# zengxianyu/sketchedit

Measured on AMD Instinct MI355X. Metric: images/sec, higher is better.
Workload: dtype f32; 1 GPU; SketchEdit inference forward (netM+netG, use_cam, pool max) 256x256 batch 32 per GPU, procedural weights; global_batch=32, size=256, per_gpu_batch=32, execution=default, two streams

## Files before the change

sketchedit_amd/csrc/se_kernels.h:

```cpp
#pragma once
#include <hip/hip_runtime.h>
#include <stddef.h>
#include <stdint.h>

#include <vector>

struct se_window;

namespace se {

enum ProfLabel { PL_GCONV_N192 = 0, PL_GCONV_N96, PL_GCONV_N48, PL_GCONV_N24, PL_WINO_N192, PL_WINO_N96, PL_WINO_UP96, PL_SMALL_CONV, PL_PACK, PL_COLREDUCE,
                 PL_ATT_PREP, PL_ATT_SCORE, PL_ATT_SOFTMAX, PL_ATT_BOXSUM, PL_ATT_PV, PL_LAYOUT,
                 PL_ATT_STREAM_STATS, PL_ATT_STREAM_OUT, PL_RESIZE_H, PL_RESIZE_V, PL_WINDOW_GATHER, PL_WINDOW_BORDER, PL_WINDOW_PASTE,
                 PL_WINDOW_RESAMPLE_H, PL_WINDOW_PASTE_V, PL_WINDOW_SAVE, PL_WINDOW_SWAP, PL_WINDOW_LOCK_GATHER, PL_WINDOW_PASTE_LOCKED,
                 PL_WINDOW_PASTE_V_LOCKED, PL_SKETCH_TILES, PL_SKETCH_STROKES, PL_PNG_ROWS, PL_PNG_STRIPES,
                 PL_PNG_FINISH, PL_JPG_BLOCKS, PL_JPG_ROWS, PL_JPG_FINISH, PL_JPG2_BLOCKS, PL_JPG2_HIST, PL_JPG2_TABLES,
                 PL_WINDOW_PASTE_FEATHER, PL_FILL_MASKS, PL_FILL_KEEP, PL_BLEND_INIT, PL_BLEND_PULL, PL_BLEND_RELAX, PL_BLEND_APPLY, PL_CANVAS_MAP, PL_CANVAS_TURN,
                 PL_SELECT_SIMILAR, PL_SELECT_FLOOD, PL_SELECT_GROW, PL_MODIFY_DISC, PL_MODIFY_VOTE,
                 PL_LASSO_FILL, PL_PLANE_COMBINE, PL_ADJUST, PL_HIST_TILES, PL_HIST_SUM, PL_ADJUST_LUT, PL_OUTLINE_COUNT, PL_OUTLINE_SCAN, PL_OUTLINE_EMIT, PL_FILTER_BLUR, PL_FILTER_MOSAIC, PL_MOVE_DROP,
                 PL_PLANE_SHIFT, PL_WARP_DROP, PL_PLANE_WARP, PL_COUNT };
const char* prof_label_name(int l);
struct Profiler {
  struct Rec { int label; const char* name; const char* form; double flops; double exec_flops; double bytes; long blocks; hipEvent_t a, b; };
  std::vector<Rec> recs;
  std::vector<hipEvent_t> pool;
  size_t used = 0;
  bool on = false;
};
void set_profiler(Profiler* p);
void set_launch_cost(double flops, double bytes, const char* name = nullptr, double exec_flops = -1.0);
void set_launch_grid(long blocks);
hipError_t ensure_max_lds(const void* func, int bytes);

#define SE_OPTIONS(X)                                                                                         \
  X(XCD_REMAP, 1)                                                             \
  X(RTILE, 1)                                              \
  X(RTILE_LL_MIN, 256)         \
  X(RTILE_WX, 2)          \
  X(RTILE_DENSE, 1)                                          \
  X(RTILE_D5W, 1)                                        \
  X(TEST_OFFSET_LIMIT, 0)  \
  X(TEST_POISON, 0)       \
  X(RCONV16, 1) X(RCONV16_DUAL, 1) X(RCONV96, 1) X(VECBIAS, 1)                                                  \
  X(WINOGRAD, 1) X(WINOGRAD48, 1) X(WINOGRAD_UP, 1) X(WINOGRAD_UP48, 1)                                         \
  X(WINOGRAD_F43, 1)      \
  X(S2_POLY, 1)           \
  X(GCONV_FAST, 1) X(FORK_DEFAULT, 1) X(LL_WINO_MIN_WG, 64) X(LL_WINO48_MIN_WG, 128)                            \
  X(ATT_FUSED, -1) X(ATT_FUSED_BF16, -1) X(ATT_PTILDE_LDS, 1) X(ATT_STATS_LDS, 1) X(ATT_E16, 1) X(ATT_SYM, 1)   \
  X(ATT_STREAM, 0)        \
  X(PAIR_MIN_PIXELS, 1 << 21)
enum Opt {
#define X(name, dflt) OPT_##name,
  SE_OPTIONS(X)
#undef X
  OPT_COUNT
};
int opt(int o);
int opt_set(const char* name, int value);
int opt_get(const char* name, int* value);
void opt_reset();
long long opt_epoch();

struct GConvParams {
  const float* src0;
  const float* src1;
  const float* wpk;
  const float* bias;
  float* dst;
  const float* zeros;
  int B, Hin, Win, Ho, Wo;
  int C0, C1;
  int C0g, CG;
  int T, KW;
  int magicCG, magicKW;
  int magicKH;
  unsigned rep;
  unsigned div_hw_m, div_w_m;
  int div_hw_l, div_w_l;
  int stride, dil, pad;
  int ushift;
  int up2;
  int OH, OW;
  int Hlim, Wlim;
  int src1_vec;
  int nch;
  int G;
  int act;
  int total_pix;
  int xcd;
  int np_full;
  int nf_full;
  int bf16;
  int small_grid;
};

static inline void udiv_magic_host(unsigned d, unsigned* m, int* l) {
  int ll = 0;
  while ((1ull << ll) < d) ++ll;
  *l = ll;
  *m = (unsigned)(((1ull << 32) * ((1ull << ll) - d)) / d + 1);
}

enum GConvCfg { GC_N192 = 0, GC_N96 = 1, GC_N48 = 2, GC_N24 = 3 };
static inline int gconv_np(int cfg) { return cfg == GC_N192 ? 192 : cfg == GC_N96 ? 96 : cfg == GC_N48 ? 48 : 32; }
static inline bool gconv_mixed(int cfg) { return cfg >= GC_N48; }

hipError_t launch_gconv(int cfg, const GConvParams& p, hipStream_t st);

struct WinoParams {
  const float* src;
  const float* src1;
  int src1_vec;
  const float* upk;
  const float* bias;
  float* dst;
  int B, h, w, d;
  int th, tw;
  int total_tiles;
  int act;
  int xcd;
  unsigned div_tpi_m, div_tw_m, div_d_m;
  int div_tpi_l, div_tw_l, div_d_l;
  const float* vbias;
};
hipError_t launch_wino(const WinoParams& p, hipStream_t st);
hipError_t launch_vecbias(const float* wv, const float* vec, float* T, int B, int C1, hipStream_t st, int round_vec = 0);
hipError_t launch_wino24(const WinoParams& p, hipStream_t st);
hipError_t launch_wino24_c48(const WinoParams& p, hipStream_t st);
hipError_t launch_wino48(const WinoParams& p, hipStream_t st);
hipError_t launch_wino48_c24(const WinoParams& p, hipStream_t st);
hipError_t launch_winoup(const WinoParams& p, hipStream_t st);
hipError_t launch_winoup48(const WinoParams& p, hipStream_t st);
hipError_t launch_s2poly48(const WinoParams& p, int halves, hipStream_t st);

struct RConvParams {
  const void* src;
  const void* wpk;
  const float* bias;
  void* dst;
  int B, h, w, d;
  int hs, ws;
  int ty, tx;
  int act;
  int xcd;
  const float* vbias;
  int dual;
};
hipError_t launch_rconv16(const RConvParams& p, hipStream_t st);

struct RConv96Params {
  const void* src;
  const void* wpk;
  const float* bias;
  void* dst;
  int B, h, w;
  int CG;
  int ty, tx;
  int stride, oh, ow;
  int up2;
  int act;
  int xcd;
};
hipError_t launch_rconv96(const RConv96Params& p, hipStream_t st);

struct RTileParams {
  const float* src;
  const float* wpk;
  const float* bias;
  float* dst;
  int B, Hin, Win;
  int C;
  int CG;
  int T, KW;
  int magicCG, magicKW;
  int pad;
  int up2, OH, OW;
  int G;
  int nch, NP;
  int RH, RW;
  int raw_bytes;
  unsigned div_cg_m, div_rw_m;
  int div_cg_l, div_rw_l;
  int ty, tx;
  int act, bf16, xcd;
  int dense;
};
hipError_t launch_rtile(const RTileParams& p, hipStream_t st);
hipError_t launch_rtilew(const RTileParams& p, hipStream_t st);
hipError_t launch_rtilew2(const RTileParams& p, hipStream_t st);
int rtile_rows(bool bf16);

struct SmallConvParams {
  const float* x;
  const float* w;
  const float* b;
  int B, H, W, cout;
  int mode;
  float* out_nchw;
  float* hard;
  const float* img;
  const float* mask;
  float* xnow;
  float* composed;
  int no_mask_coarse;
  long out_bs;
  long mask_bs;
  long comp_bs;
  int bf16;
  unsigned char* rgb8;
  unsigned char* m8;
  const unsigned char* lock;
  int raw_fine;
};
hipError_t launch_small_conv(const SmallConvParams& p, hipStream_t st);

hipError_t launch_pack_m(const float* image, const float* sketch, float* dst4, int B, int H, int W, hipStream_t st);
hipError_t launch_pack_g(const float* x, const float* x2, const float* mask, const float* mask2, const float* guide,
                         float* coarse8, float* style8, int B, int H, int W, int no_mask_cc, int joint,
                         hipStream_t st);
hipError_t launch_nchw_to_nhwc(const float* src, float* dst, int B, int C, int Cpad, int H, int W, hipStream_t st);
hipError_t launch_dequantize_u8(const unsigned char* rgb, const unsigned char* sk8, const float* lut, float* image, float* sketch,
                                int B, int H, int W, hipStream_t st);
hipError_t launch_nhwc_to_nchw(const float* src, float* dst, int B, int C, int Cstride, int H, int W, hipStream_t st);
hipError_t launch_quantize_u8(const float* composed, const float* mask, unsigned char* rgb, unsigned char* m8, int B, int H,
                              int W, hipStream_t st);
hipError_t launch_colreduce(const float* x, float* partial, float* out, int B, int HW, int C, int op, hipStream_t st,
                            int x_bf16 = 0, float* out_bf16 = nullptr);
hipError_t launch_pack_m16(const float* image, const float* sketch, float* dst8, int B, int H, int W, hipStream_t st);
hipError_t launch_pack_g16(const float* x, const float* x2, const float* mask, const float* mask2, const float* guide,
                           float* coarse8, float* style8, int B, int H, int W, int no_mask_cc, int joint, hipStream_t st);
hipError_t launch_nchw_to_nhwc16(const float* src, float* dst, int B, int C, int Cpad, int H, int W, hipStream_t st);
hipError_t launch_nhwc16_to_nchw(const float* src, float* dst, int B, int C, int Cstride, int H, int W, hipStream_t st);
static const int COLREDUCE_SPLITS = 128;

struct AttParams {
  const float* x;
  const float* rn;
  float* xn;
  const float* hard;
  float* valid;
  float* S;
  float* out;
  int B, h, w, hs, ws, L, Lp;
  float scale;
  float th;
  int hc, wc, R, Rp;
  float* xT;
  float* E;
  float* P;
  float* Pt;
  float* stats;
  float* kmul;
  float* kadd;
  int guard;
  float* validR;
  float* similar;
  int bf16;
  int e16;
  float* emean;
  float* epart;
  float* ea;
  float* eb;
  float* ea4;
  float* kadd2;
  int sym;
  int symT;
};
hipError_t launch_attention(const AttParams& p, hipStream_t st);
hipError_t launch_att2_prep(const AttParams& p, hipStream_t st);
hipError_t launch_attention_stream(const AttParams& p, hipStream_t st);
int att_stream_xt_tail();

int resample_ksize(int in, int out, int filter);
int resample_coeffs(int in, int out, int filter, int* bounds, int* kk);
enum { RESIZE_OUT_U8 = 0, RESIZE_OUT_IMAGE_F32 = 1, RESIZE_OUT_SKETCH_F32 = 2, RESIZE_OUT_LOCK_U8 = 3 };
struct ResizeOut {
  int mode;
  unsigned char* u8;
  float* f32;
  const float* lut;
  int H, W;
};
hipError_t launch_resample_h(const unsigned char* in, const int* d_bounds, const int* d_kk, const int* h_bounds, int ksize,
                             int B, int Hrows, int Win, int Wout, int C, const ResizeOut& o, hipStream_t st);
hipError_t launch_resample_v(const unsigned char* in, const int* d_bounds, const int* d_kk, int ksize, int B, int Hin, int Hout,
                             int W, int C, const ResizeOut& o, hipStream_t st);
hipError_t launch_window_resample_h(const se_window* d_wins, const int* d_bounds, const int* d_kk, const int* h_bounds, int ksize,
                                    int B, int hs, int ws, int Wout, int C, const ResizeOut& o, hipStream_t st);
hipError_t launch_window_paste_v(const se_window* d_wins, const unsigned char* rgb, const unsigned char* m8, const int* d_bounds,
                                 const int* d_kk, int ksize, int B, int Hin, int hs, int P, int ws, hipStream_t st, bool locked = false);
hipError_t launch_window_lock_resample_h(const se_window* d_wins, const int* d_bounds, const int* d_kk, const int* h_bounds, int ksize,
                                         int B, int hs, int ws, int Wout, const ResizeOut& o, hipStream_t st);
constexpr int RESAMPLE_MAX_KSIZE = 8191;

hipError_t launch_window_gather(const se_window* d_wins, const float* lut, float* image, float* sketch, int B, int H, int W,
                                hipStream_t st);
hipError_t launch_window_border(const se_window* d_wins, const unsigned char* m8, int* hits, int B, int H, int W, int hs, int ws,
                                hipStream_t st);
hipError_t launch_window_paste(const se_window* d_wins, const unsigned char* rgb, const unsigned char* m8, int B, int H, int W,
                               hipStream_t st, bool locked = false);
hipError_t launch_window_paste_feather(const se_window* d_wins, const unsigned char* rgb, const unsigned char* m8, int B, int hs, int ws,
                                       int radius, hipStream_t st);
hipError_t launch_window_lock_gather(const se_window* d_wins, unsigned char* out, int B, int H, int W, hipStream_t st);
hipError_t launch_window_journal(const se_window* d_wins, int B, int hs, int ws, bool swap, hipStream_t st);
hipError_t launch_sketch_tiles(const unsigned char* plane, int Hi, int Wi, int tile, int* tiles_out, hipStream_t st);
hipError_t launch_sketch_strokes(const se_window* d_wins, int B, int hs, int ws, const int* segs, long nseg_sum, unsigned char* sketch_out,
                                 hipStream_t st);
hipError_t launch_fill_masks(const unsigned char* fill, const unsigned char* lock, float* hole, float* hard, float* zero, int B, int H,
                             int W, hipStream_t st);
hipError_t launch_fill_keep(const se_window* d_wins, int B, int hs, int ws, hipStream_t st);
hipError_t launch_select_similar(const unsigned char* frame, int Hi, int Wi, int seed_y, int seed_x, int tolerance, int contiguous,
                                 unsigned char* state, hipStream_t st);
hipError_t launch_select_flood(unsigned char* state, int Hi, int Wi, unsigned* changed, hipStream_t st);
hipError_t launch_select_grow(const unsigned char* state, int Hi, int Wi, int grow, unsigned char* out, hipStream_t st);
hipError_t launch_plane_modify(const unsigned char* plane, int Hi, int Wi, int op, int radius, unsigned char* out, hipStream_t st);
hipError_t launch_lasso_fill(const int* edges, int N, int Hi, int Wi, unsigned char* plane_out, hipStream_t st);
hipError_t launch_plane_combine(const unsigned char* a, const unsigned char* b, int Hi, int Wi, int op, unsigned char* out, hipStream_t st);
hipError_t launch_outline_count(const unsigned char* plane, int Hi, int Wi, int* cnt, hipStream_t st);
hipError_t launch_outline_scan(int* cnt, int Hi, int Wi, int cap, int* info_out, hipStream_t st);
hipError_t launch_outline_emit(const unsigned char* plane, int Hi, int Wi, const int* offs, int* edges_out, int cap, hipStream_t st);
hipError_t launch_move_drop(unsigned char* frame, int Hi, int Wi, const unsigned char* lift, int ly0, int lx0, int lw, int lpitch,
                            const unsigned char* sel, const unsigned char* lock, int by0, int bx0, int by1, int bx1, int dy, int dx, int flip,
                            int radius, hipStream_t st);
hipError_t launch_plane_shift(const unsigned char* sel, int Hi, int Wi, int by0, int bx0, int by1, int bx1, int dy, int dx, int flip,
                              unsigned char* out, hipStream_t st);
size_t blend_workspace_bytes(int eh, int ew);
hipError_t launch_move_blend(unsigned char* frame, int Hi, int Wi, const unsigned char* lift, int ly0, int lx0, int lh, int lw, int lpitch,
                             const unsigned char* sel, const unsigned char* lock, int by0, int bx0, int by1, int bx1, int dy, int dx, int flip,
                             void* ws, hipStream_t st);
hipError_t launch_canvas(const unsigned char* in, int Hi, int Wi, int C, unsigned char* out, int Hn, int Wn, int oy, int ox, int orient,
                         int pad, unsigned rgb, hipStream_t st);
hipError_t launch_filter_blur(unsigned char* frame, int Hi, int Wi, const unsigned char* lift, int ly0, int lx0, int lw, int lpitch,
                              const unsigned char* sel, const unsigned char* lock, int by0, int bx0, int by1, int bx1, const int* taps,
                              int radius, int amount, int feather, hipStream_t st);
hipError_t launch_filter_mosaic(unsigned char* frame, int Hi, int Wi, const unsigned char* lift, int ly0, int lx0, int lw, int lpitch,
                                const unsigned char* sel, const unsigned char* lock, int by0, int bx0, int by1, int bx1, int cell, int amount,
                                int feather, hipStream_t st);
int adjust_hist_groups(int bh, int bw);
hipError_t launch_adjust(unsigned char* frame, int Hi, int Wi, const unsigned char* lift, int ly0, int lx0, int lw, int lpitch,
                         const unsigned char* sel, const unsigned char* lock, int by0, int bx0, int by1, int bx1, const unsigned char* lut,
                         const int* matrix, int amount, int feather, hipStream_t st);
hipError_t launch_hist_tiles(const unsigned char* frame, int Wi, const unsigned char* sel, int by0, int bx0, int by1, int bx1, unsigned* slabs,
                             hipStream_t st);
hipError_t launch_hist_sum(const unsigned* slabs, int groups, unsigned* hist, hipStream_t st);
hipError_t launch_adjust_lut(const unsigned* hist_src, const unsigned* hist_ref, int mode, int which, int clip, unsigned char* lut, hipStream_t st);
hipError_t launch_warp_drop(unsigned char* frame, int Hi, int Wi, const unsigned char* lift, int ly0, int lx0, int lw, int lpitch,
                            const unsigned char* sel, const unsigned char* lock, int by0, int bx0, int by1, int bx1, int ry0, int rx0,
                            int rh, int rw, const long long* m, hipStream_t st);
hipError_t launch_plane_warp(const unsigned char* sel, int Hi, int Wi, int by0, int bx0, int by1, int bx1, const long long* m,
                             unsigned char* out, hipStream_t st);
int png_stripes(int hs);
size_t png_stripe_bound(size_t n);
size_t png_slot_bytes(int ws);
hipError_t launch_png_rows(const se_window* d_wins, int B, int hs, int ws, unsigned char* ftype, hipStream_t st);
hipError_t launch_png_stripes(const se_window* d_wins, int B, int hs, int ws, const unsigned char* ftype, unsigned* sizes, unsigned* parts,
                              unsigned char* slots, hipStream_t st);
hipError_t launch_png_finish(int B, int hs, int ws, const unsigned* sizes, const unsigned* parts, const unsigned char* slots, unsigned char* out,
                             size_t cap, unsigned long long* sizes_out, hipStream_t st);
int jpg_rows(int hs, int flags);
int jpg_row_blocks(int ws, int flags);
size_t jpg_row_bound(int nblk, int flags);
size_t jpg_slot_bytes(int nblk, int flags);
hipError_t launch_jpg_blocks(const se_window* d_wins, int B, int hs, int ws, int quality, short* coef, hipStream_t st);
hipError_t launch_jpg2_blocks420(const se_window* d_wins, int B, int hs, int ws, int quality, short* coef, hipStream_t st);
hipError_t launch_jpg2_hist(int B, int R, int nblk, int flags, const short* coef, unsigned* hist, hipStream_t st);
hipError_t launch_jpg2_tables(int B, int R, const unsigned* hist, unsigned* codes, unsigned char* tables_out, hipStream_t st);
hipError_t launch_jpg_rows(int B, int R, int nblk, int flags, const short* coef, const unsigned* codes, unsigned* sizes,
                           unsigned char* slots, hipStream_t st);
hipError_t launch_jpg_finish(int B, int R, int nblk, size_t slot_bytes, const unsigned* sizes, const unsigned char* slots,
                             unsigned char* out, size_t cap, unsigned long long* sizes_out, hipStream_t st);

}
```

sketchedit_amd/csrc/se_s2poly.h:

```cpp
#pragma once
#include <hip/hip_runtime.h>

#include <cstddef>
#include <vector>

namespace se {

constexpr int S2POLY_NPOS = 25;
constexpr int S2POLY_NIT = 38;

__host__ __device__ constexpr int s2poly_src_a(int q) { return q == 0 ? 1 : q == 1 ? 3 : q == 2 ? 0 : 2; }
__host__ __device__ constexpr int s2poly_src_b(int q) { return q == 2 ? 2 : q == 4 ? 4 : -1; }
__host__ __device__ constexpr int s2poly_wcoef(int q, int k) { return q < 2 ? k == 1 : q == 2 ? k == 0 : q == 3 ? k != 1 : k == 2; }
__host__ __device__ constexpr int s2poly_fold(int q, int o) {
  return o == 0 ? (q == 0 || q == 2 || q == 3 ? 1 : 0) : (q == 1 || q == 3 ? 1 : q == 4 ? -1 : 0);
}

inline bool s2poly_pack_host(const float* w, const float* b, int cout, std::vector<float>& img, std::vector<float>& bias) {
  if (cout != 96 && cout != 192) return false;
  const int NP = cout, G = cout / 2;
  img.assign((size_t)(NP / 96) * S2POLY_NIT * 96 * 32, 0.f);
  bias.assign((size_t)NP, 0.f);
  for (int n = 0; n < NP; ++n) {
    const int f = n / 16 * 8 + n % 8, oc = n % 16 < 8 ? f : G + f;
    const int hf = n / 96, r = n % 96;
    bias[n] = b[oc];
    for (int ic = 0; ic < 48; ++ic) {
      const float* g = w + ((size_t)oc * 48 + ic) * 9;
      for (int pos = 0; pos < S2POLY_NPOS; ++pos) {
        const int py = pos / 5, px = pos % 5;
        double u = 0.;
        for (int ky = 0; ky < 3; ++ky)
          for (int kx = 0; kx < 3; ++kx) u += (double)(s2poly_wcoef(py, ky) * s2poly_wcoef(px, kx)) * (double)g[ky * 3 + kx];
        const int pp = pos >> 1, u6 = (pos & 1) * 3 + ic / 16;
        const int it = pp * 3 + u6 / 2, kin = (u6 % 2) * 16 + ic % 16;
        const int slot = (kin / 4) ^ ((r >> 1) & 7);
        img[(((size_t)hf * S2POLY_NIT + it) * 96 + r) * 32 + slot * 4 + kin % 4] = (float)u;
      }
    }
  }
  return true;
}

}
```

sketchedit_amd/csrc/se_s2poly.hip:

```cpp
#include "se_device.h"
#include "se_s2poly.h"

#include <cstdlib>
#include <type_traits>

namespace se {

template <int I, int N, typename F>
DEVFN void static_for_s2(F&& f) {
  if constexpr (I < N) {
    f(std::integral_constant<int, I>{});
    static_for_s2<I + 1, N>(f);
  }
}

__global__ __launch_bounds__(256, 2) void s2poly48_kernel(const WinoParams p) {
  constexpr int TILES = 64, NTHR = 256, NWV = 4;
  constexpr int XB = TILES * 128, WB = 96 * 128;
  constexpr int NPOS = S2POLY_NPOS, NIT = S2POLY_NIT;
  constexpr unsigned PSB = 192;
  extern __shared__ __attribute__((aligned(16))) char smem[];
  char* Xb = smem;
  char* Wb = smem + 3 * XB;

  const int tid = threadIdx.x, lane = tid & 63;
  const float eluw = p.act == 0 ? 1.f : 0.f;
  const int w = __builtin_amdgcn_readfirstlane(tid >> 6);
  const int chh = w & 1, tp = w >> 1;
  const int half = (int)blockIdx.y;
  const int tile_base = (p.xcd ? xcd_tile(blockIdx.x, gridDim.x) : (int)blockIdx.x) * TILES;
  const int tpi = p.th * p.tw;
  const float* upk = p.upk + (size_t)half * NIT * 96 * 32;
  const float* bias = p.bias + half * 96;

  auto tile_origin = [&](int t, int& b, int& iy, int& ix) {
    b = (int)udiv_magic((unsigned)t, p.div_tpi_m, p.div_tpi_l);
    const int rem = t - b * tpi;
    iy = (int)udiv_magic((unsigned)rem, p.div_tw_m, p.div_tw_l);
    ix = rem - iy * p.tw;
  };

  const int sg = tid & 3, srow = (tid >> 6) * 16 + ((tid >> 2) & 1) * 8 + ((tid >> 3) & 7);
  const int swz = (srow >> 1) & 7;
  char* xw0 = Xb + srow * 128 + ((sg ^ swz) << 4);
  char* xw1 = Xb + srow * 128 + (((4 + sg) ^ swz) << 4);
  int* Ysrc = (int*)(smem + 3 * XB + 4 * WB);
  int* Xsrc = Ysrc + 5 * NTHR;
  {
    const int t = tile_base + srow;
    int b, iy, ix;
    tile_origin(t < p.total_tiles ? t : 0, b, iy, ix);
#pragma unroll
    for (int i = 0; i < 5; ++i) {
      const int y = 4 * iy - 1 + i;
      Ysrc[i * NTHR + tid] = (t < p.total_tiles && (unsigned)y < (unsigned)p.h) ? (int)((unsigned)((b * p.h + y) * p.w) * PSB + (unsigned)sg * 16u) : (int)(0x80000000u + (unsigned)sg * 16u);
    }
    if (tid < TILES) {
      const int t2 = tile_base + tid;
      tile_origin(t2 < p.total_tiles ? t2 : 0, b, iy, ix);
#pragma unroll
      for (int i = 0; i < 5; ++i) {
        const int x = 4 * ix - 1 + i;
        Xsrc[i * TILES + tid] = ((unsigned)x < (unsigned)p.w) ? x * (int)PSB : (int)0x80000000;
      }
    }
  }
  __syncthreads();
  const unsigned lds_w = lds_addr_of(Wb);
  int off0, off1;
  frag_offsets(lane, off0, off1);

  auto need = [&](int pos, int i) {
    if (pos >= NPOS) return false;
    return !((i >= 2 && s2poly_src_b(pos / 5) < 0) || ((i & 1) && s2poly_src_b(pos % 5) < 0));
  };
  unsigned o[2][4];
  auto set_pos = [&](int set, int pos) {
    const int py = pos / 5, px = pos % 5;
    const unsigned ya = (unsigned)Ysrc[s2poly_src_a(py) * NTHR + tid], xa = (unsigned)Xsrc[s2poly_src_a(px) * TILES + srow];
    o[set][0] = __builtin_elementwise_add_sat(ya, xa);
    if (s2poly_src_b(px) >= 0) o[set][1] = __builtin_elementwise_add_sat(ya, (unsigned)Xsrc[s2poly_src_b(px) * TILES + srow]);
    if (s2poly_src_b(py) >= 0) {
      const unsigned yb = (unsigned)Ysrc[s2poly_src_b(py) * NTHR + tid];
      o[set][2] = __builtin_elementwise_add_sat(yb, xa);
      if (s2poly_src_b(px) >= 0) o[set][3] = __builtin_elementwise_add_sat(yb, (unsigned)Xsrc[s2poly_src_b(px) * TILES + srow]);
    }
  };
  auto half_set = [](int it, int h) { return (it % 3) * 2 + h >= 3 ? 1 : 0; };
  auto half_grp = [](int it, int h) { return ((it % 3) * 2 + h) % 3; };
  auto half_pos = [&](int it, int h) { return 2 * (it / 3) + half_set(it, h); };
  const __amdgpu_buffer_rsrc_t rs0 = __builtin_amdgcn_make_buffer_rsrc((void*)p.src, 0, (int)((unsigned)p.B * (unsigned)p.h * (unsigned)p.w * PSB), 0x00020000);
  auto load_x1 = [&](int it, f32x4 (&r)[2][4], int h, int i) {
    typedef unsigned u32x4 __attribute__((ext_vector_type(4)));
    if (need(half_pos(it, h), i))
      r[h][i] = __builtin_bit_cast(f32x4, (u32x4)__builtin_amdgcn_raw_buffer_load_b128(rs0, (int)o[half_set(it, h)][i], half_grp(it, h) * 64, 0));
  };
  float negone = -1.f;
  asm volatile("" : "+v"(negone));
  auto signed_sum = [&](const f32x4 (&q)[4], int pos) -> f32x4 {
    f32x4 ps = q[0], ns = {0.f, 0.f, 0.f, 0.f};
    bool hn = false;
    if (need(pos, 3)) ps = ps + q[3];
#pragma unroll
    for (int i = 1; i < 3; ++i)
      if (need(pos, i)) { ns = hn ? ns + q[i] : q[i]; hn = true; }
    return hn ? ns * negone + ps : ps;
  };
  auto write_x = [&](int it, int buf, const f32x4 (&r)[2][4]) {
    *(f32x4*)(xw0 + buf * XB) = signed_sum(r[0], half_pos(it, 0));
    if (half_pos(it, 1) < NPOS) *(f32x4*)(xw1 + buf * XB) = signed_sum(r[1], half_pos(it, 1));
  };
  auto dma_w = [&](int it, int buf, int j) {
    const int rbk = j * NWV + w;
    glds16_s(upk + (size_t)it * 96 * 32 + rbk * 256, (unsigned)lane * 16u, lds_w + buf * WB + rbk * 1024);
  };

  f32x4 am[3][2];
  f32x4 oy[2][2][3][2];
#pragma unroll
  for (int j = 0; j < 3; ++j)
#pragma unroll
    for (int q = 0; q < 2; ++q) {
      am[j][q] = (f32x4){0.f, 0.f, 0.f, 0.f};
      const f32x4 b4 = *(const f32x4*)(bias + (3 * chh + j) * 16 + (lane >> 4) * 4);
#pragma unroll
      for (int a = 0; a < 2; ++a)
#pragma unroll
        for (int b = 0; b < 2; ++b) oy[a][b][j][q] = b4;
    }
  float neg1 = -1.f;
  asm volatile("" : "+v"(neg1));
  auto fold = [&](int pos) {
    const int py = pos / 5, px = pos % 5;
    const int ay[2] = {s2poly_fold(py, 0), s2poly_fold(py, 1)};
    const int ax[2] = {s2poly_fold(px, 0), s2poly_fold(px, 1)};
#pragma unroll
    for (int j = 0; j < 3; ++j)
#pragma unroll
      for (int q = 0; q < 2; ++q) {
#pragma unroll
        for (int a = 0; a < 2; ++a)
#pragma unroll
          for (int b = 0; b < 2; ++b) {
            const int c = ay[a] * ax[b];
            if (c > 0) oy[a][b][j][q] += am[j][q];
            else if (c < 0) oy[a][b][j][q] = am[j][q] * neg1 + oy[a][b][j][q];
          }
        asm volatile("" : "+v"(oy[0][0][j][q]), "+v"(oy[0][1][j][q]), "+v"(oy[1][0][j][q]), "+v"(oy[1][1][j][q]));
      }
  };

  auto end_barrier = [&]() {
    __builtin_amdgcn_sched_barrier(0);
    asm volatile("s_waitcnt lgkmcnt(0)\n\ts_barrier" ::: "memory");
    __builtin_amdgcn_sched_barrier(0);
  };

  f32x4 r[2][4];
  set_pos(0, 0);
  set_pos(1, 1);
#pragma unroll
  for (int i0 = 0; i0 < 3; ++i0) { dma_w(i0, i0, 0); dma_w(i0, i0, 1); dma_w(i0, i0, 2); }
  {
    f32x4 r1[2][4];
#pragma unroll
    for (int i = 0; i < 4; ++i) { load_x1(0, r, 0, i); load_x1(0, r, 1, i); }
#pragma unroll
    for (int i = 0; i < 4; ++i) { load_x1(1, r1, 0, i); load_x1(1, r1, 1, i); }
    write_x(0, 0, r);
    write_x(1, 1, r1);
  }
  set_pos(0, 2);
  dma_wait_all();
  __syncthreads();
#pragma unroll
  for (int i = 0; i < 4; ++i) { load_x1(2, r, 0, i); load_x1(2, r, 1, i); }

  const char* Xw = Xb + tp * 32 * 128;
  const char* Ww = Wb + (3 * chh) * 2048;
  f32x4 wa[3], xa[2];
  xa[0] = *(const f32x4*)(Xw + off0);
  xa[1] = *(const f32x4*)(Xw + 2048 + off0);
#pragma unroll
  for (int j = 0; j < 3; ++j) wa[j] = *(const f32x4*)(Ww + j * 2048 + off0);

  static_for_s2<0, NIT>([&](auto it_c) __attribute__((always_inline)) {
    constexpr int it = decltype(it_c)::value;
    constexpr int pp = it / 3, c = it % 3;
    constexpr int b0 = it % 3, b1 = (it + 1) % 3, b2 = (it + 2) % 3;
    constexpr int w0 = it % 4, w1 = (it + 1) % 4, w3 = (it + 3) % 4;
    constexpr bool more1 = it + 1 < NIT, more2 = it + 2 < NIT, more3 = it + 3 < NIT;
    constexpr bool second = 2 * pp + (c >= 1 ? 1 : 0) < NPOS;
    f32x4 wb[3], xb[2];
    if (second) {
      xb[0] = *(const f32x4*)(Xw + b0 * XB + off1);
      xb[1] = *(const f32x4*)(Xw + b0 * XB + 2048 + off1);
#pragma unroll
      for (int j = 0; j < 3; ++j) wb[j] = *(const f32x4*)(Ww + w0 * WB + j * 2048 + off1);
    }
    __builtin_amdgcn_sched_barrier(0);
    auto group = [&](const f32x4 (&wf)[3], const f32x4 (&xf)[2], int e, bool first) {
#pragma unroll
      for (int j = 0; j < 3; ++j)
#pragma unroll
        for (int q = 0; q < 2; ++q) {
          const f32x4 cin = first ? (f32x4){0.f, 0.f, 0.f, 0.f} : am[j][q];
          am[j][q] = __builtin_amdgcn_mfma_f32_16x16x4f32(wf[j][e], xf[q][e], cin, 0, 0, 0);
        }
      __builtin_amdgcn_sched_barrier(0);
    };
    if (c == 0 && it > 0) {
      fold(2 * pp - 1);
      __builtin_amdgcn_sched_barrier(0);
    }
    group(wa, xa, 0, c == 0);
    group(wa, xa, 1, false);
    group(wa, xa, 2, false);
    group(wa, xa, 3, false);
    if (c == 1) {
      fold(2 * pp);
      __builtin_amdgcn_sched_barrier(0);
    }
    if (more2) {
      dma_wait_all();
      write_x(it + 2, b2, r);
    }
    if (c == 2 && 2 * (pp + 2) < NPOS) set_pos(0, 2 * (pp + 2));
    if (c == 0 && 2 * (pp + 1) + 1 < NPOS) set_pos(1, 2 * (pp + 1) + 1);
    __builtin_amdgcn_sched_barrier(0);
    if (second) group(wb, xb, 0, c == 1);
    if (more3) { dma_w(it + 3, w3, 0); load_x1(it + 3, r, 0, 0); load_x1(it + 3, r, 0, 1); }
    if (more1) {
      xa[0] = *(const f32x4*)(Xw + b1 * XB + off0);
      xa[1] = *(const f32x4*)(Xw + b1 * XB + 2048 + off0);
#pragma unroll
      for (int j = 0; j < 3; ++j) wa[j] = *(const f32x4*)(Ww + w1 * WB + j * 2048 + off0);
    }
    __builtin_amdgcn_sched_barrier(0);
    if (second) group(wb, xb, 1, false);
    if (more3) { dma_w(it + 3, w3, 1); load_x1(it + 3, r, 0, 2); load_x1(it + 3, r, 0, 3); }
    __builtin_amdgcn_sched_barrier(0);
    if (second) group(wb, xb, 2, false);
    if (more3) { dma_w(it + 3, w3, 2); load_x1(it + 3, r, 1, 0); load_x1(it + 3, r, 1, 1); }
    __builtin_amdgcn_sched_barrier(0);
    if (second) group(wb, xb, 3, false);
    if (more3) { load_x1(it + 3, r, 1, 2); load_x1(it + 3, r, 1, 3); }
    if (more1) end_barrier();
  });

  const int q = lane >> 4;
  const int OH = p.h >> 1, OW = p.w >> 1;
  const unsigned pix_bytes = 192u * gridDim.y;
#pragma unroll
  for (int tq = 0; tq < 2; ++tq) {
    const int t = tile_base + tp * 32 + tq * 16 + (lane & 15);
    int b = 0, iy = 0, ix = 0;
    tile_origin(t < p.total_tiles ? t : 0, b, iy, ix);
#pragma unroll
    for (int j = 0; j < 3; ++j) {
      const int c0 = half * 48 + (3 * chh + j) * 8 + (q & 1) * 4 + (q >> 1) * 2;
#pragma unroll
      for (int a = 0; a < 2; ++a)
#pragma unroll
        for (int bb = 0; bb < 2; ++bb) {
          const f32x4 v = oy[a][bb][j][tq];
          const auto s02 = __builtin_amdgcn_permlane32_swap(__float_as_uint(v[0]), __float_as_uint(v[2]), false, false);
          const auto s13 = __builtin_amdgcn_permlane32_swap(__float_as_uint(v[1]), __float_as_uint(v[3]), false, false);
          const float f0 = __uint_as_float(s02[0]), g0 = __uint_as_float(s02[1]);
          const float f1 = __uint_as_float(s13[0]), g1 = __uint_as_float(s13[1]);
          float2 ov;
          ov.x = act_fast(f0, eluw) * sigmoid_fast(g0);
          ov.y = act_fast(f1, eluw) * sigmoid_fast(g1);
          if (t < p.total_tiles)
            *(float2*)((char*)p.dst + ((unsigned)((b * OH + 2 * iy + a) * OW + 2 * ix + bb) * pix_bytes + (unsigned)c0 * 4u)) = ov;
        }
    }
  }
}

hipError_t launch_s2poly48(const WinoParams& p, int halves, hipStream_t st) {
  constexpr int TILES = 64;
  constexpr int LDS = 3 * TILES * 128 + 4 * 96 * 128 + 5 * TILES * 4 * 4 + 5 * TILES * 4;
  static_assert(LDS <= 80 * 1024, "two workgroups per CU");
  if ((halves != 1 && halves != 2) || (p.h % 4) || (p.w % 4) || p.th != p.h / 4 || p.tw != p.w / 4) return hipErrorInvalidValue;
  if ((double)p.B * p.h * p.w * 192.0 >= 2147483648.0) return hipErrorInvalidValue;
  {
    hipError_t e = ensure_max_lds((const void*)s2poly48_kernel, LDS);
    if (e != hipSuccess) return e;
  }
  const int grid = (p.total_tiles + TILES - 1) / TILES;
  set_launch_grid((long)grid * halves);
  ProfScope ps_(st, PL_WINO_N96, "s2poly48");
  hipLaunchKernelGGL(s2poly48_kernel, dim3(grid, halves), dim3(TILES * 4), LDS, st, p);
  return hipGetLastError();
}

}
```

sketchedit_amd/kernel_labels.py:

```python

KERNEL_LABELS = {
    "wino_kernel": "wino_n192", "wino24_kernel": "wino_n192", "rconv16": "gconv_n192", "gconv_kernel<12": "gconv_n192",
    "wino48_kernel": "wino_n96", "rconv96": "gconv_n96", "gconv_kernel<6": "gconv_n96",
    "s2poly48_kernel": "wino_n96",
    "winoup_kernel": "wino_up96",
    "winoup48_kernel": "gconv_n48", "rtile_dense5w_kernel": "gconv_n48", "rtile_dense5_kernel": "gconv_n48",
    "rtile_kernel<3": "gconv_n48", "gconv_kernel<3": "gconv_n48",
    "rtilew2_kernel": "gconv_n24", "rtilew_kernel": "gconv_n24", "rtile_kernel<2": "gconv_n24", "gconv_kernel<2": "gconv_n24",
    "dtail_kernel": "dtail",
    "att2_pair_kernel": "att_score", "att2_pv_kernel": "att_pv",
    "att2_softmax": "att_softmax", "att2_stats": "att_softmax",
    "att2_boxsum": "att_boxsum", "att2_ptilde": "att_boxsum",
    "att2_prep": "att_prep", "att2_transpose": "att_prep", "att2_emean": "att_prep", "att2_eoff": "att_prep",
    "att2_similar": "layout",
    "small_conv_kernel": "small_conv", "pack_": "pack", "colreduce": "colreduce", "vecbias_kernel": "colreduce",
    "nchw_to_nhwc": "layout", "nhwc_to_nchw": "layout", "nhwc16_to_nchw": "layout", "quantize_u8_kernel": "layout",
    "dequant_u8_kernel": "layout",
    "(anonymous namespace)::window_resample_h_kernel": "window_resample_h", "(anonymous namespace)::window_paste_v_kernel": "window_paste_v",
    "window_resample_h_kernel": "window_resample_h", "window_paste_v_kernel": "window_paste_v",
    "(anonymous namespace)::resample_h_kernel": "resize_h", "(anonymous namespace)::resample_v_kernel": "resize_v",
    "resample_h_kernel": "resize_h", "resample_v_kernel": "resize_v",
    "(anonymous namespace)::window_gather_kernel": "window_gather", "(anonymous namespace)::window_border_kernel": "window_border",
    "(anonymous namespace)::window_paste_kernel": "window_paste",
    "window_gather_kernel": "window_gather", "window_border_kernel": "window_border", "window_paste_kernel": "window_paste",
    "(anonymous namespace)::window_paste_feather_kernel": "window_paste_feather", "window_paste_feather_kernel": "window_paste_feather",
    "(anonymous namespace)::fill_masks_kernel": "fill_masks", "(anonymous namespace)::fill_keep_kernel": "fill_keep",
    "fill_masks_kernel": "fill_masks", "fill_keep_kernel": "fill_keep",
    "(anonymous namespace)::select_similar_kernel": "select_similar", "(anonymous namespace)::select_flood_kernel": "select_flood",
    "(anonymous namespace)::select_grow_kernel": "select_grow",
    "select_similar_kernel": "select_similar", "select_flood_kernel": "select_flood", "select_grow_kernel": "select_grow",
    "(anonymous namespace)::modify_disc_kernel": "modify_disc", "(anonymous namespace)::modify_vote_kernel": "modify_vote",
    "modify_disc_kernel": "modify_disc", "modify_vote_kernel": "modify_vote",
    "(anonymous namespace)::lasso_fill_kernel": "lasso_fill", "(anonymous namespace)::plane_combine_kernel": "plane_combine",
    "lasso_fill_kernel": "lasso_fill", "plane_combine_kernel": "plane_combine",
    "(anonymous namespace)::outline_tile_kernel<false>": "outline_count", "(anonymous namespace)::outline_tile_kernel<true>": "outline_emit",
    "(anonymous namespace)::outline_scan_kernel": "outline_scan",
    "outline_tile_kernel<false>": "outline_count", "outline_tile_kernel<true>": "outline_emit", "outline_scan_kernel": "outline_scan",
    "(anonymous namespace)::move_drop_kernel<false>": "move_drop", "(anonymous namespace)::move_drop_kernel<true>": "move_drop",
    "(anonymous namespace)::plane_shift_kernel": "plane_shift",
    "move_drop_kernel<false>": "move_drop", "move_drop_kernel<true>": "move_drop", "plane_shift_kernel": "plane_shift",
    "(anonymous namespace)::blend_init_kernel": "blend_init", "(anonymous namespace)::blend_pull_kernel": "blend_pull",
    "(anonymous namespace)::blend_relax_kernel": "blend_relax", "(anonymous namespace)::blend_apply_kernel": "blend_apply",
    "blend_init_kernel": "blend_init", "blend_pull_kernel": "blend_pull", "blend_relax_kernel": "blend_relax",
    "blend_apply_kernel": "blend_apply",
    "(anonymous namespace)::canvas_map_kernel": "canvas_map", "(anonymous namespace)::canvas_turn_kernel": "canvas_turn",
    "canvas_map_kernel": "canvas_map", "canvas_turn_kernel": "canvas_turn",
    "(anonymous namespace)::warp_drop_kernel": "warp_drop", "(anonymous namespace)::plane_warp_kernel": "plane_warp",
    "warp_drop_kernel": "warp_drop", "plane_warp_kernel": "plane_warp",
    "(anonymous namespace)::filter_blur_kernel<8>": "filter_blur", "(anonymous namespace)::filter_blur_kernel<16>": "filter_blur",
    "(anonymous namespace)::filter_blur_kernel<32>": "filter_blur", "(anonymous namespace)::filter_mosaic_kernel": "filter_mosaic",
    "filter_blur_kernel<8>": "filter_blur", "filter_blur_kernel<16>": "filter_blur", "filter_blur_kernel<32>": "filter_blur",
    "filter_mosaic_kernel": "filter_mosaic",
    "(anonymous namespace)::adjust_kernel": "adjust", "(anonymous namespace)::hist_tiles_kernel": "hist_tiles",
    "(anonymous namespace)::hist_sum_kernel": "hist_sum", "(anonymous namespace)::adjust_lut_kernel": "adjust_lut",
    "adjust_kernel": "adjust", "hist_tiles_kernel": "hist_tiles", "hist_sum_kernel": "hist_sum", "adjust_lut_kernel": "adjust_lut",
    "(anonymous namespace)::window_save_kernel": "window_save", "(anonymous namespace)::window_swap_kernel": "window_swap",
    "window_save_kernel": "window_save", "window_swap_kernel": "window_swap",
    "(anonymous namespace)::sketch_tiles_kernel": "sketch_tiles", "sketch_tiles_kernel": "sketch_tiles",
    "(anonymous namespace)::sketch_strokes_kernel": "sketch_strokes", "sketch_strokes_kernel": "sketch_strokes",
    "(anonymous namespace)::png_rows_kernel": "png_rows", "(anonymous namespace)::png_stripe_kernel": "png_stripes",
    "(anonymous namespace)::png_finish_kernel": "png_finish",
    "png_rows_kernel": "png_rows", "png_stripe_kernel": "png_stripes", "png_finish_kernel": "png_finish",
    "(anonymous namespace)::jpg_blocks_kernel": "jpg_blocks", "(anonymous namespace)::jpg_rows_kernel": "jpg_rows",
    "(anonymous namespace)::jpg_finish_kernel": "jpg_finish",
    "jpg_blocks_kernel": "jpg_blocks", "jpg_rows_kernel": "jpg_rows", "jpg_finish_kernel": "jpg_finish",
    "(anonymous namespace)::jpg2_blocks420_kernel": "jpg2_blocks420", "(anonymous namespace)::jpg2_hist_kernel": "jpg2_hist",
    "(anonymous namespace)::jpg2_tables_kernel": "jpg2_tables", "(anonymous namespace)::jpg2_rows_kernel": "jpg2_rows",
    "jpg2_blocks420_kernel": "jpg2_blocks420", "jpg2_hist_kernel": "jpg2_hist", "jpg2_tables_kernel": "jpg2_tables",
    "jpg2_rows_kernel": "jpg2_rows",
}


def kernel_key(name):
    return name.split("(")[0].replace("void se::", "").replace("se::", "")


def label_of(name):
    k = kernel_key(name)
    return next((v for pre, v in KERNEL_LABELS.items() if k.startswith(pre)), None)
```

Before: 3060 images/sec.

## Fuse both output-channel halves of s2poly conv into one 512-thread workgroup

```diff
diff --git a/sketchedit_amd/csrc/se_kernels.h b/sketchedit_amd/csrc/se_kernels.h
--- a/sketchedit_amd/csrc/se_kernels.h
+++ b/sketchedit_amd/csrc/se_kernels.h
@@ -45,6 +45,7 @@
   X(WINOGRAD, 1) X(WINOGRAD48, 1) X(WINOGRAD_UP, 1) X(WINOGRAD_UP48, 1)                                         \
   X(WINOGRAD_F43, 1)      \
   X(S2_POLY, 1)           \
+  X(S2_POLY_JOINT, 1)     \
   X(GCONV_FAST, 1) X(FORK_DEFAULT, 1) X(LL_WINO_MIN_WG, 64) X(LL_WINO48_MIN_WG, 128)                            \
   X(ATT_FUSED, -1) X(ATT_FUSED_BF16, -1) X(ATT_PTILDE_LDS, 1) X(ATT_STATS_LDS, 1) X(ATT_E16, 1) X(ATT_SYM, 1)   \
   X(ATT_STREAM, 0)        \
diff --git a/sketchedit_amd/csrc/se_s2poly.h b/sketchedit_amd/csrc/se_s2poly.h
--- a/sketchedit_amd/csrc/se_s2poly.h
+++ b/sketchedit_amd/csrc/se_s2poly.h
@@ -15,6 +15,13 @@
 __host__ __device__ constexpr int s2poly_fold(int q, int o) {
   return o == 0 ? (q == 0 || q == 2 || q == 3 ? 1 : 0) : (q == 1 || q == 3 ? 1 : q == 4 ? -1 : 0);
 }
+
+__host__ __device__ constexpr int s2poly_half_set(int it, int h) { return (it % 3) * 2 + h >= 3 ? 1 : 0; }
+__host__ __device__ constexpr int s2poly_half_grp(int it, int h) { return ((it % 3) * 2 + h) % 3; }
+__host__ __device__ constexpr int s2poly_half_pos(int it, int h) { return 2 * (it / 3) + s2poly_half_set(it, h); }
+__host__ __device__ constexpr int s2poly192_group(int it) { return it & 1; }
+__host__ __device__ constexpr int s2poly192_granule(int tid) { return tid & 3; }
+__host__ __device__ constexpr int s2poly192_tile(int tid) { return ((tid >> 6) & 3) * 16 + ((tid >> 2) & 1) * 8 + ((tid >> 3) & 7); }
 
 inline bool s2poly_pack_host(const float* w, const float* b, int cout, std::vector<float>& img, std::vector<float>& bias) {
   if (cout != 96 && cout != 192) return false;
diff --git a/sketchedit_amd/csrc/se_s2poly.hip b/sketchedit_amd/csrc/se_s2poly.hip
--- a/sketchedit_amd/csrc/se_s2poly.hip
+++ b/sketchedit_amd/csrc/se_s2poly.hip
@@ -278,17 +278,302 @@
   }
 }
 
+__global__ __launch_bounds__(512) void s2poly192_kernel(const WinoParams p) {
+  constexpr int TILES = 64, NTASK = 256, NWV = 4;
+  constexpr int XB = TILES * 128, WB = 96 * 128;
+  constexpr int NPOS = S2POLY_NPOS, NIT = S2POLY_NIT;
+  constexpr unsigned PSB = 192;
+  extern __shared__ __attribute__((aligned(16))) char smem[];
+  char* Xb = smem;
+  char* Wb = smem + 3 * XB;
+
+  const int tid = threadIdx.x, lane = tid & 63, task = tid & (NTASK - 1);
+  const float eluw = p.act == 0 ? 1.f : 0.f;
+  const int w8 = __builtin_amdgcn_readfirstlane(tid >> 6);
+  const int half = w8 >> 2, w = w8 & 3;
+  const int chh = w & 1, tp = w >> 1;
+  const int tile_base = (p.xcd ? xcd_tile(blockIdx.x, gridDim.x) : (int)blockIdx.x) * TILES;
+  const int tpi = p.th * p.tw;
+  const float* upk = p.upk + (size_t)half * NIT * 96 * 32;
+  const float* bias = p.bias + half * 96;
+
+  auto tile_origin = [&](int t, int& b, int& iy, int& ix) {
+    b = (int)udiv_magic((unsigned)t, p.div_tpi_m, p.div_tpi_l);
+    const int rem = t - b * tpi;
+    iy = (int)udiv_magic((unsigned)rem, p.div_tw_m, p.div_tw_l);
+    ix = rem - iy * p.tw;
+  };
+
+  const int sg = s2poly192_granule(tid), srow = s2poly192_tile(tid);
+  const int swz = (srow >> 1) & 7;
+  char* xw0 = Xb + srow * 128 + ((sg ^ swz) << 4);
+  char* xw1 = Xb + srow * 128 + (((4 + sg) ^ swz) << 4);
+  int* Ysrc = (int*)(smem + 3 * XB + 8 * WB);
+  int* Xsrc = Ysrc + 5 * NTASK;
+  if (tid < NTASK) {
+    const int t = tile_base + srow;
+    int b, iy, ix;
+    tile_origin(t < p.total_tiles ? t : 0, b, iy, ix);
+#pragma unroll
+    for (int i = 0; i < 5; ++i) {
+      const int y = 4 * iy - 1 + i;
+      Ysrc[i * NTASK + tid] = (t < p.total_tiles && (unsigned)y < (unsigned)p.h) ? (int)((unsigned)((b * p.h + y) * p.w) * PSB + (unsigned)sg * 16u) : (int)(0x80000000u + (unsigned)sg * 16u);
+    }
+    if (tid < TILES) {
+      const int t2 = tile_base + tid;
+      tile_origin(t2 < p.total_tiles ? t2 : 0, b, iy, ix);
+#pragma unroll
+      for (int i = 0; i < 5; ++i) {
+        const int x = 4 * ix - 1 + i;
+        Xsrc[i * TILES + tid] = ((unsigned)x < (unsigned)p.w) ? x * (int)PSB : (int)0x80000000;
+      }
+    }
+  }
+  __syncthreads();
+  const unsigned lds_w = lds_addr_of(Wb + half * 4 * WB);
+  int off0, off1;
+  frag_offsets(lane, off0, off1);
+
+  auto need = [&](int pos, int i) {
+    if (pos >= NPOS) return false;
+    return !((i >= 2 && s2poly_src_b(pos / 5) < 0) || ((i & 1) && s2poly_src_b(pos % 5) < 0));
+  };
+  unsigned o[2][4];
+  auto set_pos = [&](int set, int pos) {
+    const int py = pos / 5, px = pos % 5;
+    const unsigned ya = (unsigned)Ysrc[s2poly_src_a(py) * NTASK + task], xa = (unsigned)Xsrc[s2poly_src_a(px) * TILES + srow];
+    o[set][0] = __builtin_elementwise_add_sat(ya, xa);
+    if (s2poly_src_b(px) >= 0) o[set][1] = __builtin_elementwise_add_sat(ya, (unsigned)Xsrc[s2poly_src_b(px) * TILES + srow]);
+    if (s2poly_src_b(py) >= 0) {
+      const unsigned yb = (unsigned)Ysrc[s2poly_src_b(py) * NTASK + task];
+      o[set][2] = __builtin_elementwise_add_sat(yb, xa);
+      if (s2poly_src_b(px) >= 0) o[set][3] = __builtin_elementwise_add_sat(yb, (unsigned)Xsrc[s2poly_src_b(px) * TILES + srow]);
+    }
+  };
+  const int src_bytes = __builtin_amdgcn_readfirstlane((int)((unsigned)p.B * (unsigned)p.h * (unsigned)p.w * PSB));
+  const __amdgpu_buffer_rsrc_t rs0 = __builtin_amdgcn_make_buffer_rsrc((void*)p.src, 0, src_bytes, 0x00020000);
+  auto load_x1 = [&](int it, f32x4 (&r)[2][4], int h, int i) {
+    typedef unsigned u32x4 __attribute__((ext_vector_type(4)));
+    if (need(s2poly_half_pos(it, h), i))
+      r[h][i] = __builtin_bit_cast(f32x4, (u32x4)__builtin_amdgcn_raw_buffer_load_b128(rs0, (int)o[s2poly_half_set(it, h)][i], s2poly_half_grp(it, h) * 64, 0));
+  };
+  float negone = -1.f;
+  asm volatile("" : "+v"(negone));
+  auto signed_sum = [&](const f32x4 (&q)[4], int pos) -> f32x4 {
+    f32x4 ps = q[0], ns = {0.f, 0.f, 0.f, 0.f};
+    bool hn = false;
+    if (need(pos, 3)) ps = ps + q[3];
+#pragma unroll
+    for (int i = 1; i < 3; ++i)
+      if (need(pos, i)) { ns = hn ? ns + q[i] : q[i]; hn = true; }
+    return hn ? ns * negone + ps : ps;
+  };
+  auto write_x = [&](int it, int buf, const f32x4 (&r)[2][4]) {
+    *(f32x4*)(xw0 + buf * XB) = signed_sum(r[0], s2poly_half_pos(it, 0));
+    if (s2poly_half_pos(it, 1) < NPOS) *(f32x4*)(xw1 + buf * XB) = signed_sum(r[1], s2poly_half_pos(it, 1));
+  };
+  auto dma_w = [&](int it, int buf, int j) {
+    const int rbk = j * NWV + w;
+    glds16_s(upk + (size_t)it * 96 * 32 + rbk * 256, (unsigned)lane * 16u, lds_w + buf * WB + rbk * 1024);
+  };
+
+  f32x4 am[3][2];
+  f32x4 oy[2][2][3][2];
+#pragma unroll
+  for (int j = 0; j < 3; ++j)
+#pragma unroll
+    for (int q = 0; q < 2; ++q) {
+      am[j][q] = (f32x4){0.f, 0.f, 0.f, 0.f};
+      const f32x4 b4 = *(const f32x4*)(bias + (3 * chh + j) * 16 + (lane >> 4) * 4);
+#pragma unroll
+      for (int a = 0; a < 2; ++a)
+#pragma unroll
+        for (int b = 0; b < 2; ++b) oy[a][b][j][q] = b4;
+    }
+  float neg1 = -1.f;
+  asm volatile("" : "+v"(neg1));
+  auto fold = [&](int pos) {
+    const int py = pos / 5, px = pos % 5;
+    const int ay[2] = {s2poly_fold(py, 0), s2poly_fold(py, 1)};
+    const int ax[2] = {s2poly_fold(px, 0), s2poly_fold(px, 1)};
+#pragma unroll
+    for (int j = 0; j < 3; ++j)
+#pragma unroll
+      for (int q = 0; q < 2; ++q) {
+#pragma unroll
+        for (int a = 0; a < 2; ++a)
+#pragma unroll
+          for (int b = 0; b < 2; ++b) {
+            const int c = ay[a] * ax[b];
+            if (c > 0) oy[a][b][j][q] += am[j][q];
+            else if (c < 0) oy[a][b][j][q] = am[j][q] * neg1 + oy[a][b][j][q];
+          }
+        asm volatile("" : "+v"(oy[0][0][j][q]), "+v"(oy[0][1][j][q]), "+v"(oy[1][0][j][q]), "+v"(oy[1][1][j][q]));
+      }
+  };
+
+  auto mine = [&](int it) { return half == s2poly192_group(it); };
+  auto end_barrier = [&]() {
+    __builtin_amdgcn_sched_barrier(0);
+    asm volatile("s_waitcnt lgkmcnt(0)\n\ts_barrier" ::: "memory");
+    __builtin_amdgcn_sched_barrier(0);
+  };
+
+  f32x4 r[2][4];
+  set_pos(0, 0);
+  set_pos(1, 1);
+#pragma unroll
+  for (int i0 = 0; i0 < 3; ++i0) { dma_w(i0, i0, 0); dma_w(i0, i0, 1); dma_w(i0, i0, 2); }
+  if (mine(0)) {
+#pragma unroll
+    for (int i = 0; i < 4; ++i) { load_x1(0, r, 0, i); load_x1(0, r, 1, i); }
+    write_x(0, 0, r);
+  } else {
+#pragma unroll
+    for (int i = 0; i < 4; ++i) { load_x1(1, r, 0, i); load_x1(1, r, 1, i); }
+    write_x(1, 1, r);
+  }
+  set_pos(0, 2);
+  dma_wait_all();
+  __syncthreads();
+  if (mine(2)) {
+#pragma unroll
+    for (int i = 0; i < 4; ++i) { load_x1(2, r, 0, i); load_x1(2, r, 1, i); }
+  }
+
+  const char* Xw = Xb + tp * 32 * 128;
+  const char* Ww = Wb + half * 4 * WB + (3 * chh) * 2048;
+  f32x4 wa[3], xa[2];
+  xa[0] = *(const f32x4*)(Xw + off0);
+  xa[1] = *(const f32x4*)(Xw + 2048 + off0);
+#pragma unroll
+  for (int j = 0; j < 3; ++j) wa[j] = *(const f32x4*)(Ww + j * 2048 + off0);
+
+  static_for_s2<0, NIT>([&](auto it_c) __attribute__((always_inline)) {
+    constexpr int it = decltype(it_c)::value;
+    constexpr int pp = it / 3, c = it % 3;
+    constexpr int b0 = it % 3, b1 = (it + 1) % 3, b2 = (it + 2) % 3;
+    constexpr int w0 = it % 4, w1 = (it + 1) % 4, w3 = (it + 3) % 4;
+    constexpr bool more1 = it + 1 < NIT, more2 = it + 2 < NIT, more3 = it + 3 < NIT;
+    constexpr bool second = 2 * pp + (c >= 1 ? 1 : 0) < NPOS;
+    f32x4 wb[3], xb[2];
+    if (second) {
+      xb[0] = *(const f32x4*)(Xw + b0 * XB + off1);
+      xb[1] = *(const f32x4*)(Xw + b0 * XB + 2048 + off1);
+#pragma unroll
+      for (int j = 0; j < 3; ++j) wb[j] = *(const f32x4*)(Ww + w0 * WB + j * 2048 + off1);
+    }
+    __builtin_amdgcn_sched_barrier(0);
+    auto group = [&](const f32x4 (&wf)[3], const f32x4 (&xf)[2], int e, bool first) {
+#pragma unroll
+      for (int j = 0; j < 3; ++j)
+#pragma unroll
+        for (int q = 0; q < 2; ++q) {
+          const f32x4 cin = first ? (f32x4){0.f, 0.f, 0.f, 0.f} : am[j][q];
+          am[j][q] = __builtin_amdgcn_mfma_f32_16x16x4f32(wf[j][e], xf[q][e], cin, 0, 0, 0);
+        }
+      __builtin_amdgcn_sched_barrier(0);
+    };
+    if (c == 0 && it > 0) {
+      fold(2 * pp - 1);
+      __builtin_amdgcn_sched_barrier(0);
+    }
+    group(wa, xa, 0, c == 0);
+    group(wa, xa, 1, false);
+    group(wa, xa, 2, false);
+    group(wa, xa, 3, false);
+    if (c == 1) {
+      fold(2 * pp);
+      __builtin_amdgcn_sched_barrier(0);
+    }
+    if (more2) {
+      dma_wait_all();
+      if (mine(it + 2)) write_x(it + 2, b2, r);
+    }
+    if (c == 2 && 2 * (pp + 2) < NPOS) set_pos(0, 2 * (pp + 2));
+    if (c == 0 && 2 * (pp + 1) + 1 < NPOS) set_pos(1, 2 * (pp + 1) + 1);
+    __builtin_amdgcn_sched_barrier(0);
+    if (second) group(wb, xb, 0, c == 1);
+    if (more3) {
+      dma_w(it + 3, w3, 0);
+      if (mine(it + 3)) { load_x1(it + 3, r, 0, 0); load_x1(it + 3, r, 0, 1); }
+    }
+    if (more1) {
+      xa[0] = *(const f32x4*)(Xw + b1 * XB + off0);
+      xa[1] = *(const f32x4*)(Xw + b1 * XB + 2048 + off0);
+#pragma unroll
+      for (int j = 0; j < 3; ++j) wa[j] = *(const f32x4*)(Ww + w1 * WB + j * 2048 + off0);
+    }
+    __builtin_amdgcn_sched_barrier(0);
+    if (second) group(wb, xb, 1, false);
+    if (more3) {
+      dma_w(it + 3, w3, 1);
+      if (mine(it + 3)) { load_x1(it + 3, r, 0, 2); load_x1(it + 3, r, 0, 3); }
+    }
+    __builtin_amdgcn_sched_barrier(0);
+    if (second) group(wb, xb, 2, false);
+    if (more3) {
+      dma_w(it + 3, w3, 2);
+      if (mine(it + 3)) { load_x1(it + 3, r, 1, 0); load_x1(it + 3, r, 1, 1); }
+    }
+    __builtin_amdgcn_sched_barrier(0);
+    if (second) group(wb, xb, 3, false);
+    if (more3 && mine(it + 3)) { load_x1(it + 3, r, 1, 2); load_x1(it + 3, r, 1, 3); }
+    if (more1) end_barrier();
+  });
+
+  const int q = lane >> 4;
+  const int OH = p.h >> 1, OW = p.w >> 1;
+  constexpr unsigned pix_bytes = 192u * 2u;
+#pragma unroll
+  for (int tq = 0; tq < 2; ++tq) {
+    const int t = tile_base + tp * 32 + tq * 16 + (lane & 15);
+    int b = 0, iy = 0, ix = 0;
+    tile_origin(t < p.total_tiles ? t : 0, b, iy, ix);
+#pragma unroll
+    for (int j = 0; j < 3; ++j) {
+      const int c0 = half * 48 + (3 * chh + j) * 8 + (q & 1) * 4 + (q >> 1) * 2;
+#pragma unroll
+      for (int a = 0; a < 2; ++a)
+#pragma unroll
+        for (int bb = 0; bb < 2; ++bb) {
+          const f32x4 v = oy[a][bb][j][tq];
+          const auto s02 = __builtin_amdgcn_permlane32_swap(__float_as_uint(v[0]), __float_as_uint(v[2]), false, false);
+          const auto s13 = __builtin_amdgcn_permlane32_swap(__float_as_uint(v[1]), __float_as_uint(v[3]), false, false);
+          const float f0 = __uint_as_float(s02[0]), g0 = __uint_as_float(s02[1]);
+          const float f1 = __uint_as_float(s13[0]), g1 = __uint_as_float(s13[1]);
+          float2 ov;
+          ov.x = act_fast(f0, eluw) * sigmoid_fast(g0);
+          ov.y = act_fast(f1, eluw) * sigmoid_fast(g1);
+          if (t < p.total_tiles)
+            *(float2*)((char*)p.dst + ((unsigned)((b * OH + 2 * iy + a) * OW + 2 * ix + bb) * pix_bytes + (unsigned)c0 * 4u)) = ov;
+        }
+    }
+  }
+}
+
 hipError_t launch_s2poly48(const WinoParams& p, int halves, hipStream_t st) {
   constexpr int TILES = 64;
   constexpr int LDS = 3 * TILES * 128 + 4 * 96 * 128 + 5 * TILES * 4 * 4 + 5 * TILES * 4;
+  constexpr int LDS2 = 3 * TILES * 128 + 2 * 4 * 96 * 128 + 5 * TILES * 4 * 4 + 5 * TILES * 4;
   static_assert(LDS <= 80 * 1024, "two workgroups per CU");
+  static_assert(LDS2 <= 160 * 1024, "one workgroup per CU");
   if ((halves != 1 && halves != 2) || (p.h % 4) || (p.w % 4) || p.th != p.h / 4 || p.tw != p.w / 4) return hipErrorInvalidValue;
   if ((double)p.B * p.h * p.w * 192.0 >= 2147483648.0) return hipErrorInvalidValue;
+  const int grid = (p.total_tiles + TILES - 1) / TILES;
+  if (halves == 2 && opt(OPT_S2_POLY_JOINT) != 0) {
+    if (ensure_max_lds((const void*)s2poly192_kernel, LDS2) == hipSuccess) {
+      set_launch_grid((long)grid);
+      ProfScope ps_(st, PL_WINO_N96, "s2poly48");
+      hipLaunchKernelGGL(s2poly192_kernel, dim3(grid), dim3(TILES * 8), LDS2, st, p);
+      return hipGetLastError();
+    }
+    (void)hipGetLastError();
+  }
   {
     hipError_t e = ensure_max_lds((const void*)s2poly48_kernel, LDS);
     if (e != hipSuccess) return e;
   }
-  const int grid = (p.total_tiles + TILES - 1) / TILES;
   set_launch_grid((long)grid * halves);
   ProfScope ps_(st, PL_WINO_N96, "s2poly48");
   hipLaunchKernelGGL(s2poly48_kernel, dim3(grid, halves), dim3(TILES * 4), LDS, st, p);
diff --git a/sketchedit_amd/kernel_labels.py b/sketchedit_amd/kernel_labels.py
--- a/sketchedit_amd/kernel_labels.py
+++ b/sketchedit_amd/kernel_labels.py
@@ -2,7 +2,7 @@
 KERNEL_LABELS = {
     "wino_kernel": "wino_n192", "wino24_kernel": "wino_n192", "rconv16": "gconv_n192", "gconv_kernel<12": "gconv_n192",
     "wino48_kernel": "wino_n96", "rconv96": "gconv_n96", "gconv_kernel<6": "gconv_n96",
-    "s2poly48_kernel": "wino_n96",
+    "s2poly48_kernel": "wino_n96", "s2poly192_kernel": "wino_n96",
     "winoup_kernel": "wino_up96",
     "winoup48_kernel": "gconv_n48", "rtile_dense5w_kernel": "gconv_n48", "rtile_dense5_kernel": "gconv_n48",
     "rtile_kernel<3": "gconv_n48", "gconv_kernel<3": "gconv_n48",
```

Result: no change. 3052 images/sec (-0.3%).
